# dedis/kyber

Measured on AMD Instinct MI355X. Metric: scalar-muls/s + pairings/s per node; MSM sec at 2^20 points, higher is better.
Workload: dtype int32 limbs (radix 2^25.5), int64 accumulate; 1 GPU; Ed25519 batched fixed-base + var-base scalar-mul, 2^20 scalars per GPU (BASELINE.json configs[1]); elements_per_gpu=1048576

## Files before the change

kyber_amd/csrc/ed25519.hip:

```cpp
#ifndef KYB_TU_WAVES
#define KYB_TU_WAVES 2
#endif
#include "context.h"
#include "ed25519_dev.cuh"
#include "ed25519_launch.h"
#include "msm.cuh"
#include "ed25519_h2c.cuh"
#include <stdlib.h>
#include <string.h>

#include <algorithm>
#include <atomic>
#include <chrono>
#include <thread>
#include <vector>

namespace kyb {


template <int G = 2>
__global__ void ed25519_build_base_table_kernel(int32_t* __restrict__ tab, const uint32_t* __restrict__ point,
                                                uint32_t* __restrict__ ok, int rows = ED_TAB_POS * ED_TAB_ENT) {
    const int t = blockIdx.x * blockDim.x + threadIdx.x;
    if (t >= rows) return;
    ge_p3 B;
    if (point) {
        uint32_t pw[8];
        load_words8(pw, point);
        const bool good = ge_p3_fromwords(B, pw);
        if (t == 0) *ok = good ? 1u : 0u;
    } else {
        B.X = fe_bx(); B.Y = fe_by(); fe_1(B.Z); B.T = fe_bt();
    }
    ed_comb_row<G>(tab + (size_t)t * ED_TAB_STRIDE, t, B);
}

__global__ __launch_bounds__(ED_ENC_BLOCK, KYB_TU_WAVES) void ed25519_encode_kernel(size_t n, const int32_t* __restrict__ proj,
                                                            const uint8_t* __restrict__ status,
                                                            uint32_t* __restrict__ out) {
    __shared__ int32_t pre_lds[EncPreLds<ED_ENC_BLOCK>::WORDS];
    static_assert(ED_ENC_BLOCK % 64 == 0 && sizeof(pre_lds) <= 80 * 1024 && sizeof(pre_lds) / (ED_ENC_BLOCK / 64) * 4 <= 160 * 1024,
                  "LDS: at least two blocks on a CU, and a wave on every SIMD");
    EncPreLds<ED_ENC_BLOCK> pre{pre_lds + threadIdx.x};
    ed_encode_chunk(n, proj, ed_encode_first(), blockDim.x, pre, [&](size_t i, uint32_t (&w)[8]) {
        if (status && status[i]) {
#pragma unroll
            for (int k = 0; k < 8; k++) w[k] = 0;
        }
        store_words8(out + i * 8, w);
    });
}


template <int G>
__global__ __launch_bounds__(256, 3) void ed25519_mul_base_kernel(
    size_t n, const uint32_t* __restrict__ scalars, uint32_t* __restrict__ out,
    const int32_t* __restrict__ tab, uint32_t flags, int32_t* __restrict__ proj) {
    const bool full = (flags & KYB_F_VARTIME) != 0;
    for (size_t idx = (size_t)blockIdx.x * blockDim.x + threadIdx.x; idx < n;
         idx += (size_t)gridDim.x * blockDim.x) {
        uint32_t a[8];
        load_words8(a, scalars + idx * 8);
        int8_t e[65];
        recode16(e, a, full);
        ge_p3 h;
        ge_p3_0(h);
        ge_precomp t;
        ge_p1p1 r;
        const int npos = full ? EdComb<G>::POS : EdComb<G>::POS_CT;
        EdCombDigits<G> digits(e);
#pragma unroll 1
        for (int k = 0; k < npos; k++) {
            const int d = digits.next(k);
            if (full && __ballot(d != 0) == 0) continue;
            select_precomp_tab<EdComb<G>::ENT>(t, tab, k, d);
            ge_madd(r, h, t);
            ge_p1p1_to_p3(h, r);
        }
        if (proj) {
            store_proj(proj, idx, h);
            continue;
        }
        uint32_t w[8];
        ge_p3_towords(w, h);
        store_words8(out + idx * 8, w);
    }
}

KYB_DEV void select_precomp_uniform(ge_precomp& t, const int32_t* __restrict__ tab, int i, int b) {
    const bool neg = b < 0;
    const int babs = neg ? -b : b;
    const int pos = i >> 1, mult = (i & 1) ? 16 : 1;
    fe_1(t.ypx);
    fe_1(t.ymx);
    fe_0(t.xy2d);
#pragma unroll 1
    for (int m = 1; m <= 8; m++) {
        const int4* e = reinterpret_cast<const int4*>(tab + (size_t)(pos * ED_TAB_ENT + (m * mult - 1)) * ED_TAB_STRIDE);
        int32_t w[32];
#pragma unroll
        for (int q = 0; q < 8; q++) {
            const int4 x = e[q];
            w[4 * q] = x.x;
            w[4 * q + 1] = x.y;
            w[4 * q + 2] = x.z;
            w[4 * q + 3] = x.w;
        }
        const int32_t keep = -(int32_t)(babs == m);
#pragma unroll
        for (int l = 0; l < 10; l++) {
            t.ypx.v[l] ^= (t.ypx.v[l] ^ w[l]) & keep;
            t.ymx.v[l] ^= (t.ymx.v[l] ^ w[10 + l]) & keep;
            t.xy2d.v[l] ^= (t.xy2d.v[l] ^ w[20 + l]) & keep;
        }
    }
    ge_precomp_cneg(t, neg);
}
__global__ __launch_bounds__(256, 3) void ed25519_mul_base_uniform_kernel(
    size_t n, const uint32_t* __restrict__ scalars, uint32_t* __restrict__ out,
    const int32_t* __restrict__ tab, int32_t* __restrict__ proj) {
    for (size_t idx = (size_t)blockIdx.x * blockDim.x + threadIdx.x; idx < n;
         idx += (size_t)gridDim.x * blockDim.x) {
        uint32_t a[8];
        load_words8(a, scalars + idx * 8);
        int8_t e[65];
        recode16(e, a, false);
        ge_p3 h;
        ge_p3_0(h);
        ge_precomp t;
        ge_p1p1 r;
        EdCombDigits<1> digits(e);
#pragma unroll 1
        for (int i = 0; i < 64; i++) {
            select_precomp_uniform(t, tab, i, digits.next(i));
            ge_madd(r, h, t);
            ge_p1p1_to_p3(h, r);
        }
        if (proj) {
            store_proj(proj, idx, h);
            continue;
        }
        uint32_t w[8];
        ge_p3_towords(w, h);
        store_words8(out + idx * 8, w);
    }
}


template <bool GTAB, bool UNI = false>
__global__ __launch_bounds__(128, 3) void ed25519_mul_kernel(
    size_t n, const uint32_t* __restrict__ scalars, const uint32_t* __restrict__ points,
    size_t points_stride, uint32_t* __restrict__ out, uint8_t* __restrict__ status,
    uint32_t flags, int32_t* __restrict__ proj, int4* __restrict__ gtab) {
    const size_t idx = (size_t)blockIdx.x * blockDim.x + threadIdx.x;
    if (idx >= n) return;
    const bool full = !UNI && (flags & KYB_F_VARTIME) != 0;
    uint32_t pw[8], a[8];
    load_words8(pw, points + idx * points_stride);
    load_words8(a, scalars + idx * 8);
    ge29_p3 A;
    const bool ok = ge_p3_fromwords(A, pw);
    int8_t e[65];
    recode16(e, a, full);
    ge29_p3 h;
    const int vt_top = full ? wave_top_digit(a) : 63;
    if constexpr (GTAB) {
        TabGlobal_t<fe29> tab{gtab + idx * 80};
        ge_scalarmult_w4<UNI, true>(h, e, A, full, tab, vt_top);
    } else {
        TabScratch_t<fe29> tab;
        ge_scalarmult_w4<UNI, true>(h, e, A, full, tab, vt_top);
    }
    if (proj) {
        store_proj(proj, idx, h);
        if (status) status[idx] = ok ? KYB_ST_OK : KYB_ST_BAD_POINT;
        return;
    }
    uint32_t w[8];
    ge_p3_towords(w, h);
    if (!ok) {
#pragma unroll
        for (int i = 0; i < 8; i++) w[i] = 0;
    }
    store_words8(out + idx * 8, w);
    if (status) status[idx] = ok ? KYB_ST_OK : KYB_ST_BAD_POINT;
}

int ed25519_build_tables(DeviceCtx* ctx) {
    KYB_HIP_CHECK(hipMalloc(&ctx->ed_base_tab, ED_TAB_WORDS * sizeof(int32_t)));
    hipLaunchKernelGGL(ed25519_build_base_table_kernel<2>, dim3((ED_TAB_POS * ED_TAB_ENT + 63) / 64), dim3(64), 0,
                       nullptr, ctx->ed_base_tab, (const uint32_t*)nullptr, (uint32_t*)nullptr, ED_TAB_POS * ED_TAB_ENT);
    KYB_HIP_CHECK(hipGetLastError());
    const auto t0 = std::chrono::steady_clock::now();
    KYB_HIP_CHECK(hipMalloc(&ctx->ed_wide_tab, ED_WIDE_WORDS * sizeof(int32_t)));
    hipLaunchKernelGGL(ed25519_build_base_table_kernel<ED_COMB_G>, dim3((EdWide::ROWS + 63) / 64), dim3(64), 0, nullptr,
                       ctx->ed_wide_tab, (const uint32_t*)nullptr, (uint32_t*)nullptr, EdWide::ROWS);
    KYB_HIP_CHECK(hipGetLastError());
    KYB_HIP_CHECK(hipStreamSynchronize(nullptr));
    ctx->ed_wide_build_us = std::chrono::duration_cast<std::chrono::microseconds>(std::chrono::steady_clock::now() - t0).count();
    return KYB_OK;
}
void ed25519_free_tables(DeviceCtx* ctx) {
    if (ctx->ed_base_tab) hipFree(ctx->ed_base_tab);
    if (ctx->ed_wide_tab) hipFree(ctx->ed_wide_tab);
    ctx->ed_base_tab = ctx->ed_wide_tab = nullptr;
}

constexpr size_t ENC_DEFER_MIN = 4096;


static int launch_mul_base(DeviceCtx* ctx, size_t n, const void* d_scalars, void* d_out, uint32_t flags,
                           hipStream_t st, const int32_t* tab = nullptr) {
    const bool wide = !tab && !(flags & KYB_F_UNIFORM);
    if (!tab) tab = wide ? ctx->ed_wide_tab : ctx->ed_base_tab;
    if (n == 0) return KYB_OK;
    const int block = 256;
    size_t want = (n + block - 1) / block;
    size_t cap = (size_t)ctx->num_cu * 8;
    int grid = (int)(want < cap ? want : cap);
    EdSlab w{};
    std::lock_guard<std::recursive_mutex> enq_lock(ctx->enq_mu);
    if (n >= ENC_DEFER_MIN)
        if (int rc = ed_slab(ctx, st, ED_SLAB_MUL_BASE, n, &w)) return rc;
    if (flags & KYB_F_UNIFORM) {
        hipLaunchKernelGGL(ed25519_mul_base_uniform_kernel, dim3(grid), dim3(block), 0, st, n,
                           (const uint32_t*)d_scalars, (uint32_t*)d_out, tab, w.proj);
    } else {
        const auto kernel = wide ? ed25519_mul_base_kernel<ED_COMB_G> : ed25519_mul_base_kernel<2>;
        hipLaunchKernelGGL(kernel, dim3(grid), dim3(block), 0, st, n, (const uint32_t*)d_scalars, (uint32_t*)d_out, tab,
                           flags, w.proj);
    }
    if (w.proj)
        hipLaunchKernelGGL(ed25519_encode_kernel, ed_encode_grid(n), dim3(ED_ENC_BLOCK), 0, st, n, w.proj,
                           (const uint8_t*)nullptr, (uint32_t*)d_out);
    KYB_HIP_CHECK(hipGetLastError());
    return KYB_OK;
}
static int launch_mul(size_t n, const void* d_scalars, const void* d_points, size_t stride, void* d_out,
                      void* d_status, uint32_t flags, hipStream_t st) {
    if (n == 0) return KYB_OK;
    const int block = 128;
    size_t grid = (n + block - 1) / block;
    EdSlab w{};
    uint8_t* stat = (uint8_t*)d_status;
    DeviceCtx* ctx;
    int rc = get_ctx(&ctx);
    if (rc) return rc;
    std::lock_guard<std::recursive_mutex> enq_lock(ctx->enq_mu);
    const bool defer = n >= ENC_DEFER_MIN, uni = (flags & KYB_F_UNIFORM) != 0;
    const auto kernel = defer ? (uni ? ed25519_mul_kernel<true, true> : ed25519_mul_kernel<true, false>)
                              : (uni ? ed25519_mul_kernel<false, true> : ed25519_mul_kernel<false, false>);
    if (defer) {
        if ((rc = ed_slab(ctx, st, ed_slab_mul(stat == nullptr), n, &w))) return rc;
        if (!stat) stat = w.status;
    }
    hipLaunchKernelGGL(kernel, dim3((unsigned)grid), dim3(block), 0, st, n, (const uint32_t*)d_scalars,
                       (const uint32_t*)d_points, stride, (uint32_t*)d_out, stat, flags, w.proj, w.gtab);
    if (w.proj)
        hipLaunchKernelGGL(ed25519_encode_kernel, ed_encode_grid(n), dim3(ED_ENC_BLOCK), 0, st, n, w.proj,
                           (const uint8_t*)stat, (uint32_t*)d_out);
    KYB_HIP_CHECK(hipGetLastError());
    return KYB_OK;
}

}

using namespace kyb;

static bool ed_mul_flags_bad(uint32_t flags) {
    return (flags & ~(KYB_F_VARTIME | KYB_F_UNIFORM)) || (flags & (KYB_F_VARTIME | KYB_F_UNIFORM)) == (KYB_F_VARTIME | KYB_F_UNIFORM);
}

extern "C" {

int kyb_ed25519_mul_base_dev(size_t n, const void* d_scalars, void* d_out, uint32_t flags, void* stream) {
    if ((n && (!d_scalars || !d_out)) || ed_mul_flags_bad(flags)) {
        set_error("kyb_ed25519_mul_base_dev: bad argument");
        return KYB_E_ARG;
    }
    DeviceCtx* ctx;
    int rc = get_ctx(&ctx);
    if (rc) return rc;
    return launch_mul_base(ctx, n, d_scalars, d_out, flags, (hipStream_t)stream);
}

int kyb_ed25519_mul_dev(size_t n, const void* d_scalars, const void* d_points, void* d_out, void* d_status,
                        uint32_t flags, void* stream) {
    if ((n && (!d_scalars || !d_points || !d_out)) || ed_mul_flags_bad(flags)) {
        set_error("kyb_ed25519_mul_dev: bad argument");
        return KYB_E_ARG;
    }
    DeviceCtx* ctx;
    int rc = get_ctx(&ctx);
    if (rc) return rc;
    return launch_mul(n, d_scalars, d_points, 8, d_out, d_status, flags, (hipStream_t)stream);
}

static int mul_host(size_t n, const uint8_t* scalars, const uint8_t* points, size_t stride, uint8_t* out,
                    uint8_t* status, uint32_t flags);

int kyb_ed25519_mul_base(size_t n, const uint8_t* scalars, uint8_t* out, uint32_t flags) {
    if ((n && (!scalars || !out)) || ed_mul_flags_bad(flags)) {
        set_error("kyb_ed25519_mul_base: bad argument");
        return KYB_E_ARG;
    }
    if (n == 0) return KYB_OK;
    if (md_active(n))
        return md_run(n, [&](int, size_t lo, size_t hi) { return kyb_ed25519_mul_base(hi - lo, scalars + 32 * lo, out + 32 * lo, flags); });
    return mul_host(n, scalars, nullptr, 0, out, nullptr, flags);
}

constexpr size_t PIPE_CHUNK_MAX = PIN_SLOT_ELEMS;
constexpr int PIPE_SLOTS = DeviceCtx::NPIN, PIPE_STREAMS = 3;
static size_t pipe_chunk(const DeviceCtx* ctx) {
    if (const char* e = getenv("KYB_PIPE_CHUNK")) {
        const size_t v = (size_t)strtoull(e, nullptr, 10) & ~size_t(63);
        if (v >= 4096) return std::min(PIPE_CHUNK_MAX, v);
    }
    (void)ctx;
    return size_t(1) << 17;
}
static int pipe_nstreams() {
    if (const char* e = getenv("KYB_PIPE_STREAMS")) {
        const int v = atoi(e);
        if (v >= 1 && v <= PIPE_STREAMS) return v;
// ... 466 lines not shown
```

kyber_amd/csrc/ed25519_consts.inc:

```
KYB_DEV fe fe_d() { return fe{{56195235, 13857412, 51736253, 6949390, 114729, 24766616, 60832955, 30306712, 48412415, 21499315}}; }
KYB_DEV fe fe_d2() { return fe{{45281625, 27714825, 36363642, 13898781, 229458, 15978800, 54557047, 27058993, 29715967, 9444199}}; }
KYB_DEV fe fe_sqrtm1() { return fe{{34513072, 25610706, 9377949, 3500415, 12389472, 33281959, 41962654, 31548777, 326685, 11406482}}; }
KYB_DEV fe fe_bx() { return fe{{52811034, 25909283, 16144682, 17082669, 27570973, 30858332, 40966398, 8378388, 20764389, 8758491}}; }
KYB_DEV fe fe_by() { return fe{{40265304, 26843545, 13421772, 20132659, 26843545, 6710886, 53687091, 13421772, 40265318, 26843545}}; }
KYB_DEV fe fe_bt() { return fe{{28827043, 27438313, 39759291, 244362, 8635006, 11264893, 19351346, 13413597, 16611511, 27139452}}; }
KYB_DEV fe fe_elligator_c1() { return fe{{54885894, 25242303, 55597453, 9067496, 51808079, 33312638, 25456129, 14121551, 54921728, 3972023}}; }
KYB_DEV fe fe_elligator_c2() { return fe{{34513073, 25610706, 9377949, 3500415, 12389472, 33281959, 41962654, 31548777, 326685, 11406482}}; }
```

kyber_amd/csrc/ed25519_dev.cuh:

```cuda
#pragma once
#include "ge25519.cuh"

#if !defined(__HIPCC__)
#include <type_traits>
struct int4 { int32_t x, y, z, w; };
struct uint4 { uint32_t x, y, z, w; };
inline int4 make_int4(int32_t x, int32_t y, int32_t z, int32_t w) { return int4{x, y, z, w}; }
inline uint4 make_uint4(uint32_t x, uint32_t y, uint32_t z, uint32_t w) { return uint4{x, y, z, w}; }
#define KYB_DEV_CONST static
#else
#define KYB_DEV_CONST __device__
#endif

namespace kyb {

constexpr int ED_TAB_POS = 33;
constexpr int ED_TAB_ENT = 136;
constexpr int ED_TAB_STRIDE = 32;
constexpr int ED_TAB_WORDS = ED_TAB_POS * ED_TAB_ENT * ED_TAB_STRIDE;

template <int G>
struct EdComb {
    static constexpr int POS = (65 + G - 1) / G;
    static constexpr int POS_CT = (64 + G - 1) / G;
    static constexpr int ENT = 8 * ((1 << (4 * G)) - 1) / 15;
    static constexpr int LAST_D = 65 - G * (POS - 1);
    static constexpr int LAST_ENT = 8 * ((1 << (4 * LAST_D)) - 1) / 15;
    static constexpr int ROWS = (POS - 1) * ENT + LAST_ENT;
};
#ifndef ED_COMB_G
#define ED_COMB_G 4
#endif
using EdWide = EdComb<ED_COMB_G>;
constexpr size_t ED_WIDE_WORDS = (size_t)EdWide::ROWS * ED_TAB_STRIDE;

KYB_DEV void load_words8(uint32_t w[8], const uint32_t* __restrict__ p) {
    const uint4 a = reinterpret_cast<const uint4*>(p)[0];
    const uint4 b = reinterpret_cast<const uint4*>(p)[1];
    w[0] = a.x; w[1] = a.y; w[2] = a.z; w[3] = a.w;
    w[4] = b.x; w[5] = b.y; w[6] = b.z; w[7] = b.w;
}
KYB_DEV void store_words8(uint32_t* __restrict__ p, const uint32_t w[8]) {
    reinterpret_cast<uint4*>(p)[0] = make_uint4(w[0], w[1], w[2], w[3]);
    reinterpret_cast<uint4*>(p)[1] = make_uint4(w[4], w[5], w[6], w[7]);
}

template <int G>
KYB_DEV void ed_comb_row(int32_t* __restrict__ o, int t, const ge_p3& B) {
    constexpr int ENT = EdComb<G>::ENT;
    const int pos = t / ENT, j = t - pos * ENT;
    ge_cached cB;
    ge_p3_to_cached(cB, B);
    ge_p3 acc;
    ge_p3_0(acc);
    ge_p1p1 r;
#pragma unroll 1
    for (int bit = 4 * G - 1; bit >= 0; bit--) {
        ge_dbl(r, acc.X, acc.Y, acc.Z);
        ge_p1p1_to_p3(acc, r);
        if (((j + 1) >> bit) & 1) {
            ge_add(r, acc, cB);
            ge_p1p1_to_p3(acc, r);
        }
    }
#pragma unroll 1
    for (int k = 0; k < 4 * G * pos; k++) {
        ge_dbl(r, acc.X, acc.Y, acc.Z);
        ge_p1p1_to_p3(acc, r);
    }
    fe zi, x, y, ypx, ymx, xy2d, z;
    fe_invert(zi, acc.Z);
    fe_mul(x, acc.X, zi);
    fe_mul(y, acc.Y, zi);
    fe_add(ypx, y, x);
    fe_sub(ymx, y, x);
    fe_mul(xy2d, x, y);
    fe_mul(xy2d, xy2d, fe_d2());
    fe_1(z);
    fe_mul(ypx, ypx, z);
    fe_mul(ymx, ymx, z);
#pragma unroll
    for (int l = 0; l < 10; l++) {
        o[l] = ypx.v[l];
        o[10 + l] = ymx.v[l];
        o[20 + l] = xy2d.v[l];
    }
    o[30] = o[31] = 0;
}

constexpr int ENC_CHUNK = 16;

KYB_DEV void store_proj(int32_t* __restrict__ proj, size_t idx, const ge_p3& h) {
    int32_t* o = proj + idx * 30;
#pragma unroll
    for (int l = 0; l < 10; l++) {
        o[l] = h.X.v[l];
        o[10 + l] = h.Y.v[l];
        o[20 + l] = h.Z.v[l];
    }
}
KYB_DEV void store_proj(int32_t* __restrict__ proj, size_t idx, const ge29_p3& h) {
    ge_p3 t;
    fe29_to_fe(t.X, h.X);
    fe29_to_fe(t.Y, h.Y);
    fe29_to_fe(t.Z, h.Z);
    store_proj(proj, idx, t);
}
KYB_DEV void load_fe(fe& f, const int32_t* __restrict__ p) {
#pragma unroll
    for (int l = 0; l < 10; l++) f.v[l] = p[l];
}
struct EncPreScratch {
    fe pre[ENC_CHUNK];
    KYB_DEV void put(int j, const fe& f) { pre[j] = f; }
    KYB_DEV void get(fe& f, int j) const { f = pre[j]; }
};
template <int LANES>
struct EncPreLds {
    int32_t* col;
    static constexpr int WORDS = ENC_CHUNK * 10 * LANES;
    KYB_DEV void put(int j, const fe& f) {
#pragma unroll
        for (int l = 0; l < 10; l++) col[(j * 10 + l) * LANES] = f.v[l];
    }
    KYB_DEV void get(fe& f, int j) const {
#pragma unroll
        for (int l = 0; l < 10; l++) f.v[l] = col[(j * 10 + l) * LANES];
        KYB_FE_MAG_SET(f, 1.01);
    }
};
#if defined(__HIPCC__)
template <int GROUP = 1>
KYB_DEV size_t ed_encode_first() {
    return (size_t)blockIdx.x * blockDim.x * (ENC_CHUNK / GROUP) + threadIdx.x;
}
#endif
template <int GROUP = 1, class Pre, class Emit>
KYB_DEV void ed_encode_chunk(size_t n, const int32_t* __restrict__ proj, size_t first, size_t stride, Pre& pre, Emit emit) {
    static_assert(GROUP >= 1 && GROUP <= ENC_CHUNK, "whole records per lane");
    int cnt = 0;
#pragma unroll
    for (int r = 0; r < ENC_CHUNK / GROUP; r++) cnt += (first + r * stride < n) ? GROUP : 0;
    if (cnt == 0) return;
    auto point = [&](int j) { return (first + (size_t)(j / GROUP) * stride) * GROUP + (size_t)(j % GROUP); };
    fe z, acc;
    load_fe(acc, proj + point(0) * 30 + 20);
    pre.put(0, acc);
#pragma unroll 1
    for (int j = 1; j < cnt; j++) {
        load_fe(z, proj + point(j) * 30 + 20);
        fe_mul(acc, acc, z);
        pre.put(j, acc);
    }
    fe inv;
    fe_invert(inv, acc);
#pragma unroll 1
    for (int j = cnt - 1; j >= 0; j--) {
        const size_t i = point(j);
        fe zi, X, Y;
        load_fe(z, proj + i * 30 + 20);
        if (j > 0) {
            pre.get(zi, j - 1);
            fe_mul(zi, inv, zi);
            fe_mul(inv, inv, z);
        } else {
            zi = inv;
        }
        load_fe(X, proj + i * 30);
        load_fe(Y, proj + i * 30 + 10);
        uint32_t w[8];
        ge_encode_with_zinv(w, X, Y, zi);
        emit(i, w);
    }
}

template <int ENT>
KYB_DEV void select_precomp_tab(ge_precomp& t, const int32_t* __restrict__ tab, int pos, int b) {
    const bool neg = b < 0;
    const int babs = neg ? -b : b;
    const int4* e = reinterpret_cast<const int4*>(tab + (size_t)(pos * ENT + (babs ? babs - 1 : 0)) * ED_TAB_STRIDE);
    int32_t w[32];
#pragma unroll
    for (int i = 0; i < 8; i++) {
        const int4 x = e[i];
        w[4 * i] = x.x;
        w[4 * i + 1] = x.y;
        w[4 * i + 2] = x.z;
        w[4 * i + 3] = x.w;
    }
#pragma unroll
    for (int l = 0; l < 10; l++) {
        t.ypx.v[l] = w[l];
        t.ymx.v[l] = w[10 + l];
        t.xy2d.v[l] = w[20 + l];
    }
    if (babs == 0) {
        fe_1(t.ypx);
        fe_1(t.ymx);
        fe_0(t.xy2d);
    }
    ge_precomp_cneg(t, neg);
}

KYB_DEV void ed_pack_digits(uint32_t pk[8], const int8_t e[65]) {
#pragma unroll
    for (int j = 0; j < 8; j++) {
        pk[j] = 0;
#pragma unroll
        for (int q = 0; q < 8; q++) pk[j] |= (uint32_t)((e[8 * j + q] + 8) & 15) << (4 * q);
    }
}

template <int G>
struct EdCombDigits {
    static_assert(G >= 1 && G <= 7, "a position's digits are read from one 32-bit word");
    static constexpr int PACKED = 63 / G;
    static constexpr int TAIL = EdComb<G>::POS - PACKED;
    uint32_t pk[8];
    int tail[TAIL];
    KYB_DEV explicit EdCombDigits(const int8_t e[65]) {
        ed_pack_digits(pk, e);
#pragma unroll
        for (int t = 0; t < TAIL; t++) {
            int d = 0;
#pragma unroll
            for (int i = G - 1; i >= 0; i--)
                if (G * (PACKED + t) + i <= 64) d = 16 * d + (int)e[G * (PACKED + t) + i];
            tail[t] = d;
        }
    }
    KYB_DEV int next(int k) {
        int d = (int)(pk[0] & ((1u << (4 * G)) - 1u)) - EdComb<G>::ENT;
#pragma unroll
        for (int j = 0; j < 7; j++) pk[j] = (pk[j] >> (4 * G)) | (pk[j + 1] << (32 - 4 * G));
        pk[7] >>= 4 * G;
#pragma unroll
        for (int t = 0; t < TAIL; t++)
            if (k == PACKED + t) d = tail[t];
        return d;
    }
};

template <class F = fe>
struct TabScratch_t {
    typedef typename ge_t<F>::cached cached;
    cached tab[8];
    KYB_DEV void put(int j, const cached& c) { tab[j] = c; }
    KYB_DEV void get(cached& c, int j) const { c = tab[j]; }
};
using TabScratch = TabScratch_t<>;
template <class F = fe>
struct TabGlobal_t;
using TabGlobal = TabGlobal_t<>;
template <>
struct TabGlobal_t<fe> {
    int4* base;
    KYB_DEV void put(int j, const ge_cached& c) {
        int4* q = base + j * 10;
        const fe* f[4] = {&c.YpX, &c.YmX, &c.Z, &c.T2d};
        int32_t w[40];
#pragma unroll
        for (int k = 0; k < 4; k++)
#pragma unroll
            for (int l = 0; l < 10; l++) w[10 * k + l] = f[k]->v[l];
#pragma unroll
        for (int i = 0; i < 10; i++) q[i] = make_int4(w[4 * i], w[4 * i + 1], w[4 * i + 2], w[4 * i + 3]);
    }
    KYB_DEV void get(ge_cached& c, int j) const {
        const int4* q = base + j * 10;
        int32_t w[40];
#pragma unroll
        for (int i = 0; i < 10; i++) {
            const int4 x = q[i];
            w[4 * i] = x.x;
            w[4 * i + 1] = x.y;
            w[4 * i + 2] = x.z;
            w[4 * i + 3] = x.w;
        }
        fe* f[4] = {&c.YpX, &c.YmX, &c.Z, &c.T2d};
#pragma unroll
        for (int k = 0; k < 4; k++)
#pragma unroll
            for (int l = 0; l < 10; l++) f[k]->v[l] = w[10 * k + l];
    }
    KYB_DEV void get_signed(ge_cached& c, int b) const;
};
KYB_DEV_CONST __attribute__((aligned(16))) const int32_t ED_CACHED_IDENTITY[40] = {1, 0, 0, 0, 0, 0, 0, 0, 0, 0,
                                                                               1, 0, 0, 0, 0, 0, 0, 0, 0, 0,
                                                                               1};
KYB_DEV void TabGlobal_t<fe>::get_signed(ge_cached& c, int b) const {
    const bool neg = b < 0;
    const int babs = neg ? -b : b;
#if defined(__HIPCC__)
    typedef int32_t i32x2 __attribute__((ext_vector_type(2)));
    typedef int32_t i32x4 __attribute__((ext_vector_type(4)));
    using gint = const __attribute__((address_space(1))) int32_t;
    using gint2 = const __attribute__((address_space(1))) i32x2;
    using gint4 = const __attribute__((address_space(1))) i32x4;
#else
    struct i32x2 { int32_t x, y; };
    struct i32x4 { int32_t x, y, z, w; };
    using gint = const int32_t;
    using gint2 = const i32x2;
    using gint4 = const i32x4;
#endif
    gint* e = babs ? (gint*)(base + (babs - 1) * 10) : (gint*)ED_CACHED_IDENTITY;
    gint2* p = (gint2*)(e + (neg ? 10 : 0));
    gint2* m = (gint2*)(e + (neg ? 0 : 10));
    gint4* q = (gint4*)(e + 20);
#pragma unroll
    for (int i = 0; i < 5; i++) {
        const i32x2 x = p[i], y = m[i];
        c.YpX.v[2 * i] = x.x;
        c.YpX.v[2 * i + 1] = x.y;
        c.YmX.v[2 * i] = y.x;
        c.YmX.v[2 * i + 1] = y.y;
    }
    int32_t w[20];
#pragma unroll
    for (int i = 0; i < 5; i++) {
        const i32x4 x = q[i];
        w[4 * i] = x.x;
        w[4 * i + 1] = x.y;
        w[4 * i + 2] = x.z;
        w[4 * i + 3] = x.w;
    }
    const int32_t s = -(int32_t)neg;
#pragma unroll
    for (int l = 0; l < 10; l++) {
        c.Z.v[l] = w[l];
        c.T2d.v[l] = (w[10 + l] ^ s) - s;
    }
}
template <>
struct TabGlobal_t<fe29> {
    int4* base;
    static constexpr int word(int field, int l) { return field < 2 ? (l < 8 ? 8 * field + l : 16 + field) : 18 + 9 * (field - 2) + l; }
    KYB_DEV void put(int j, const ge29_cached& c) {
        int4* q = base + j * 9;
        const fe29* f[4] = {&c.YpX, &c.YmX, &c.Z, &c.T2d};
        int32_t w[36];
#pragma unroll
        for (int k = 0; k < 4; k++)
#pragma unroll
            for (int l = 0; l < 9; l++) w[word(k, l)] = f[k]->v[l];
#pragma unroll
        for (int i = 0; i < 9; i++) q[i] = make_int4(w[4 * i], w[4 * i + 1], w[4 * i + 2], w[4 * i + 3]);
    }
    KYB_DEV void get(ge29_cached& c, int j) const {
        const int4* q = base + j * 9;
        int32_t w[36];
#pragma unroll
        for (int i = 0; i < 9; i++) {
            const int4 x = q[i];
            w[4 * i] = x.x;
            w[4 * i + 1] = x.y;
            w[4 * i + 2] = x.z;
            w[4 * i + 3] = x.w;
        }
        fe29* f[4] = {&c.YpX, &c.YmX, &c.Z, &c.T2d};
#pragma unroll
        for (int k = 0; k < 4; k++)
#pragma unroll
            for (int l = 0; l < 9; l++) f[k]->v[l] = w[word(k, l)];
        KYB_FE_MAG_SET(c.YpX, 3.001);
        KYB_FE_MAG_SET(c.YmX, 3.001);
        KYB_FE_MAG_SET(c.Z, 1.001);
        KYB_FE_MAG_SET(c.T2d, 1.001);
    }
    KYB_DEV void get_signed(ge29_cached& c, int b) const;
};
KYB_DEV_CONST __attribute__((aligned(16))) const int32_t ED_CACHED_IDENTITY29[36] = {1, 0, 0, 0, 0, 0, 0, 0,
                                                                                 1, 0, 0, 0, 0, 0, 0, 0,
                                                                                 0, 0, 1};
KYB_DEV void TabGlobal_t<fe29>::get_signed(ge29_cached& c, int b) const {
    const bool neg = b < 0;
    const int babs = neg ? -b : b;
#if defined(__HIPCC__)
    typedef int32_t i32x4 __attribute__((ext_vector_type(4)));
    using gint = const __attribute__((address_space(1))) int32_t;
    using gint4 = const __attribute__((address_space(1))) i32x4;
#else
    struct i32x4 { int32_t x, y, z, w; };
    using gint = const int32_t;
    using gint4 = const i32x4;
#endif
    gint* e = babs ? (gint*)(base + (babs - 1) * 9) : (gint*)ED_CACHED_IDENTITY29;
    gint4* p = (gint4*)(e + (neg ? 8 : 0));
    gint4* m = (gint4*)(e + (neg ? 0 : 8));
    gint4* q = (gint4*)(e + 16);
#pragma unroll
    for (int i = 0; i < 2; i++) {
        const i32x4 x = p[i], y = m[i];
        c.YpX.v[4 * i] = x.x;
        c.YpX.v[4 * i + 1] = x.y;
        c.YpX.v[4 * i + 2] = x.z;
        c.YpX.v[4 * i + 3] = x.w;
        c.YmX.v[4 * i] = y.x;
        c.YmX.v[4 * i + 1] = y.y;
        c.YmX.v[4 * i + 2] = y.z;
        c.YmX.v[4 * i + 3] = y.w;
    }
    int32_t w[20];
#pragma unroll
    for (int i = 0; i < 5; i++) {
        const i32x4 x = q[i];
        w[4 * i] = x.x;
        w[4 * i + 1] = x.y;
        w[4 * i + 2] = x.z;
        w[4 * i + 3] = x.w;
    }
    c.YpX.v[8] = neg ? w[1] : w[0];
    c.YmX.v[8] = neg ? w[0] : w[1];
    const int32_t s = -(int32_t)neg;
#pragma unroll
    for (int l = 0; l < 9; l++) {
        c.Z.v[l] = w[2 + l];
        c.T2d.v[l] = (w[11 + l] ^ s) - s;
    }
    KYB_FE_MAG_SET(c.YpX, 3.001);
    KYB_FE_MAG_SET(c.YmX, 3.001);
    KYB_FE_MAG_SET(c.Z, 1.001);
    KYB_FE_MAG_SET(c.T2d, 1.001);
}
template <bool UNI = false, class C, class Tab>
KYB_DEV void select_cached(C& c, const Tab& tab, int b) {
    typedef decltype(c.Z) F;
    const bool neg = b < 0;
    const int babs = neg ? -b : b;
    if constexpr (UNI) {
        ge_cached_0(c);
#pragma unroll 1
        for (int m = 1; m <= 8; m++) {
            C x;
            tab.get(x, m - 1);
            const int32_t keep = -(int32_t)(babs == m);
#pragma unroll
            for (int l = 0; l < F::N; l++) {
                c.YpX.v[l] ^= (c.YpX.v[l] ^ x.YpX.v[l]) & keep;
                c.YmX.v[l] ^= (c.YmX.v[l] ^ x.YmX.v[l]) & keep;
                c.Z.v[l] ^= (c.Z.v[l] ^ x.Z.v[l]) & keep;
                c.T2d.v[l] ^= (c.T2d.v[l] ^ x.T2d.v[l]) & keep;
            }
        }
    } else if constexpr (std::is_same_v<Tab, TabGlobal_t<F>>) {
        tab.get_signed(c, b);
        return;
    } else {
        tab.get(c, babs ? babs - 1 : 0);
        if (babs == 0) ge_cached_0(c);
    }
    ge_cached_cneg(c, neg);
}

KYB_DEV int wave_top_digit(const uint32_t a[8]) {
    int bits = 0;
#pragma unroll
    for (int i = 0; i < 8; i++)
        if (a[i]) bits = 32 * i + 32 - __builtin_clz(a[i]);
    int t = (bits + 3) >> 2;
    if (t > 64) t = 64;
#if defined(__HIP_DEVICE_COMPILE__)
#pragma unroll
    for (int off = 32; off >= 1; off >>= 1) {
        const int o = __shfl_xor(t, off, 64);
        t = o > t ? o : t;
    }
    t = __builtin_amdgcn_readfirstlane(t);
#endif
    return t;
}

template <bool AFFINE = false, class P3, class Tab>
KYB_DEV void ge_window_table(Tab& tab, const P3& A) {
    typedef ge_t<decltype(A.X)> G;
    typename G::p1p1 t;
    P3 u;
    typename G::cached c;
    ge_p3_to_cached(c, A);
    tab.put(0, c);
    if constexpr (AFFINE) {
        const typename G::precomp a{c.YpX, c.YmX, c.T2d};
        u = A;
#pragma unroll 1
        for (int i = 0; i < 7; i++) {
            ge_madd(t, u, a);
            ge_p1p1_to_p3(u, t);
            ge_p3_to_cached(c, u);
            tab.put(i + 1, c);
        }
    } else {
#pragma unroll 1
        for (int i = 0; i < 7; i++) {
            ge_add(t, A, c);
            ge_p1p1_to_p3(u, t);
            ge_p3_to_cached(c, u);
            tab.put(i + 1, c);
        }
    }
}

template <bool UNI = false, bool AFFINE = false, class P3, class Tab>
KYB_DEV void ge_scalarmult_w4(P3& h, const int8_t e[65], const P3& A, bool full, Tab& tab, int vt_top) {
    typedef ge_t<decltype(A.X)> G;
    typename G::p1p1 t;
    P3 u;
    typename G::p2 r;
    typename G::cached c;
    ge_window_table<AFFINE>(tab, A);
    ge_p3_0(u);
    int top = 63;
    if (full) top = vt_top;
    select_cached<UNI>(c, tab, e[top]);
    ge_add(t, u, c);
    uint32_t pk[8];
    ed_pack_digits(pk, e);
    auto shl4 = [&pk]() {
#pragma unroll
        for (int j = 7; j > 0; j--) pk[j] = (pk[j] << 4) | (pk[j - 1] >> 28);
        pk[0] <<= 4;
    };
#pragma unroll 1
    for (int i = top; i < 64; i++) shl4();
#pragma unroll 1
    for (int i = top - 1; i >= 0; i--) {
        const int d = (int)(pk[7] >> 28) - 8;
        shl4();
        ge_p1p1_to_p2(r, t);
        ge_dbl(t, r.X, r.Y, r.Z);
        ge_p1p1_to_p2(r, t);
        ge_dbl(t, r.X, r.Y, r.Z);
        ge_p1p1_to_p2(r, t);
        ge_dbl(t, r.X, r.Y, r.Z);
        ge_p1p1_to_p2(r, t);
        ge_dbl(t, r.X, r.Y, r.Z);
#if defined(__HIP_DEVICE_COMPILE__)
        if (!UNI && full && __ballot(d != 0) == 0) continue;
#endif
        ge_p1p1_to_p3(u, t);
        select_cached<UNI>(c, tab, d);
        ge_add(t, u, c);
    }
    ge_p1p1_to_p3(h, t);
}

}
```

kyber_amd/csrc/ge25519.cuh:

```cuda
#pragma once
#include "fe25519.cuh"
#include "fe29.cuh"

namespace kyb {

struct ge_p2 { fe X, Y, Z; };
struct ge_p3 { fe X, Y, Z, T; };
struct ge_p1p1 { fe X, Y, Z, T; };
struct ge_cached { fe YpX, YmX, Z, T2d; };
struct ge_precomp { fe ypx, ymx, xy2d; };
struct ge29_p2 { fe29 X, Y, Z; };
struct ge29_p3 { fe29 X, Y, Z, T; };
struct ge29_p1p1 { fe29 X, Y, Z, T; };
struct ge29_cached { fe29 YpX, YmX, Z, T2d; };
struct ge29_precomp { fe29 ypx, ymx, xy2d; };
template <class F> struct ge_t;
template <> struct ge_t<fe> {
    typedef ge_p2 p2; typedef ge_p3 p3; typedef ge_p1p1 p1p1; typedef ge_cached cached; typedef ge_precomp precomp;
};
template <> struct ge_t<fe29> {
    typedef ge29_p2 p2; typedef ge29_p3 p3; typedef ge29_p1p1 p1p1; typedef ge29_cached cached; typedef ge29_precomp precomp;
};

#include "ed25519_consts.inc"
#include "ed25519_consts29.inc"
template <class F> struct fe_k;
template <> struct fe_k<fe> {
    static KYB_DEV fe d() { return fe_d(); }
    static KYB_DEV fe d2() { return fe_d2(); }
    static KYB_DEV fe sqrtm1() { return fe_sqrtm1(); }
};
template <> struct fe_k<fe29> {
    static KYB_DEV fe29 d() { return fe29_d(); }
    static KYB_DEV fe29 d2() { return fe29_d2(); }
    static KYB_DEV fe29 sqrtm1() { return fe29_sqrtm1(); }
};

template <class P3>
KYB_DEV void ge_p3_0(P3& h) {
    fe_0(h.X);
    fe_1(h.Y);
    fe_1(h.Z);
    fe_0(h.T);
}
template <class C>
KYB_DEV void ge_cached_0(C& c) {
    fe_1(c.YpX);
    fe_1(c.YmX);
    fe_1(c.Z);
    fe_0(c.T2d);
}
template <class P2, class P1>
KYB_DEV void ge_p1p1_to_p2(P2& r, const P1& p) {
    fe_mul(r.X, p.X, p.T);
    fe_mul(r.Y, p.Y, p.Z);
    fe_mul(r.Z, p.Z, p.T);
}
template <class P3, class P1>
KYB_DEV void ge_p1p1_to_p3(P3& r, const P1& p) {
    fe_mul(r.X, p.X, p.T);
    fe_mul(r.Y, p.Y, p.Z);
    fe_mul(r.Z, p.Z, p.T);
    fe_mul(r.T, p.X, p.Y);
}
template <class C, class P3>
KYB_DEV void ge_p3_to_cached(C& r, const P3& p) {
    fe_add(r.YpX, p.Y, p.X);
    fe_sub(r.YmX, p.Y, p.X);
    r.Z = p.Z;
    fe_mul(r.T2d, p.T, fe_k<decltype(p.T)>::d2());
}
template <class P1, class F>
KYB_DEV void ge_dbl(P1& r, const F& X, const F& Y, const F& Z) {
    F t0;
    fe_sq(r.X, X);
    fe_sq(r.Z, Y);
    fe_sq2(r.T, Z);
    fe_add(r.Y, X, Y);
    fe_sq(t0, r.Y);
    fe_add(r.Y, r.Z, r.X);
    fe_sub(r.Z, r.Z, r.X);
    fe_sub(r.X, t0, r.Y);
    fe_sub(r.T, r.T, r.Z);
}
template <class P1, class P3, class C>
KYB_DEV void ge_add(P1& r, const P3& p, const C& q) {
    decltype(p.X) t0;
    fe_add(r.X, p.Y, p.X);
    fe_sub(r.Y, p.Y, p.X);
    fe_mul(r.Z, r.X, q.YpX);
    fe_mul(r.Y, r.Y, q.YmX);
    fe_mul(r.T, q.T2d, p.T);
    fe_mul(r.X, p.Z, q.Z);
    fe_add(t0, r.X, r.X);
    fe_sub(r.X, r.Z, r.Y);
    fe_add(r.Y, r.Z, r.Y);
    fe_add(r.Z, t0, r.T);
    fe_sub(r.T, t0, r.T);
}
template <class P1, class P3, class C>
KYB_DEV void ge_madd(P1& r, const P3& p, const C& q) {
    decltype(p.X) t0;
    fe_add(r.X, p.Y, p.X);
    fe_sub(r.Y, p.Y, p.X);
    fe_mul(r.Z, r.X, q.ypx);
    fe_mul(r.Y, r.Y, q.ymx);
    fe_mul(r.T, q.xy2d, p.T);
    fe_add(t0, p.Z, p.Z);
    fe_sub(r.X, r.Z, r.Y);
    fe_add(r.Y, r.Z, r.Y);
    fe_add(r.Z, t0, r.T);
    fe_sub(r.T, t0, r.T);
}
template <class C>
KYB_DEV void ge_cached_cneg(C& c, bool neg) {
    fe_cswap(c.YpX, c.YmX, neg);
    decltype(c.T2d) nt;
    fe_neg(nt, c.T2d);
    fe_cmov(c.T2d, nt, neg);
}
KYB_DEV void ge_precomp_cneg(ge_precomp& c, bool neg) {
    fe_cswap(c.ypx, c.ymx, neg);
    fe nt;
    fe_neg(nt, c.xy2d);
    fe_cmov(c.xy2d, nt, neg);
}

template <class F>
KYB_DEV void ge_encode_with_zinv(uint32_t w[8], const F& X, const F& Y, const F& zinv) {
    F x, y;
    fe_mul(x, X, zinv);
    fe_mul(y, Y, zinv);
    fe_towords(w, y);
    w[7] ^= (uint32_t)fe_isnegative(x) << 31;
}
template <class P3>
KYB_DEV void ge_p3_towords(uint32_t w[8], const P3& p) {
    decltype(p.Z) zi;
    fe_invert(zi, p.Z);
    ge_encode_with_zinv(w, p.X, p.Y, zi);
}
template <class P3>
KYB_DEV bool ge_p3_fromwords(P3& p, const uint32_t w[8]) {
    typedef decltype(p.X) F;
    F u, v, v3, vxx, check;
    fe_fromwords(p.Y, w);
    fe_1(p.Z);
    fe_sq(u, p.Y);
    fe_mul(v, u, fe_k<F>::d());
    fe_sub(u, u, p.Z);
    fe_add(v, v, p.Z);
    fe_sq(v3, v);
    fe_mul(v3, v3, v);
    fe_sq(p.X, v3);
    fe_mul(p.X, p.X, v);
    fe_mul(p.X, p.X, u);
    fe_pow22523(p.X, p.X);
    fe_mul(p.X, p.X, v3);
    fe_mul(p.X, p.X, u);
    fe_sq(vxx, p.X);
    fe_mul(vxx, vxx, v);
    fe_sub(check, vxx, u);
    bool ok = true;
    if (fe_isnonzero(check)) {
        fe_add(check, vxx, u);
        ok = !fe_isnonzero(check);
        F xs;
        fe_mul(xs, p.X, fe_k<F>::sqrtm1());
        p.X = xs;
    }
    const bool sign = (w[7] >> 31) != 0;
    F nx;
    fe_neg(nx, p.X);
    fe_cmov(p.X, nx, fe_isnegative(p.X) != sign);
    fe_mul(p.T, p.X, p.Y);
    return ok;
}

KYB_DEV void recode16(int8_t e[65], const uint32_t a[8], bool full256) {
    int carry = 0;
#pragma unroll
    for (int i = 0; i < 64; i++) {
        int d = (int)((a[i >> 3] >> ((i & 7) * 4)) & 15) + carry;
        if (i < 63) {
            carry = (d + 8) >> 4;
            d -= carry << 4;
        }
        e[i] = (int8_t)d;
    }
    int top = e[63];
    int c2 = 0;
    if (full256) {
        c2 = (top + 8) >> 4;
        top -= c2 << 4;
    } else if (top > 8) {
        top = 0;
    }
    e[63] = (int8_t)top;
    e[64] = (int8_t)c2;
}

KYB_DEV bool ed_effective_scalar(uint32_t (&k)[8]) {
    uint32_t c = 0, t7 = 0;
#pragma unroll
    for (int j = 0; j < 8; j++) {
        const uint64_t s = (uint64_t)k[j] + (j < 7 ? 0x88888888u : 0x08888888u) + c;
        t7 = (uint32_t)s;
        c = (uint32_t)(s >> 32);
    }
    const uint32_t e63 = (c << 4) | (t7 >> 28);
    if (e63 <= 8) return false;
    const uint32_t carried = e63 - (k[7] >> 28);
    k[7] &= 0x0fffffffu;
    if (!carried) return false;
    uint32_t b = 0;
#pragma unroll
    for (int j = 0; j < 8; j++) {
        const uint64_t d = (uint64_t)(j == 7 ? 0x10000000u : 0u) - k[j] - b;
        k[j] = (uint32_t)d;
        b = (uint32_t)(d >> 63);
    }
    return true;
}

}
```

kyber_amd/csrc/gen_consts.py:

```python
#!/usr/bin/env python3
import os

HERE = os.path.dirname(os.path.abspath(__file__))


def limbs_25_5(x):
    out, off = [], 0
    for i in range(10):
        w = 25 if i & 1 else 26
        out.append((x >> off) & ((1 << w) - 1))
        off += w
    assert off == 255 and x >> 255 == 0
    return out


def ed25519():
    p = 2**255 - 19
    d = (-121665 * pow(121666, p - 2, p)) % p
    sqrtm1 = pow(2, (p - 1) // 4, p)
    by = 4 * pow(5, p - 2, p) % p
    u, v = (by * by - 1) % p, (d * by * by + 1) % p
    bx = (u * pow(v, 3, p) * pow(u * pow(v, 7, p) % p, (p - 5) // 8, p)) % p
    if (v * bx * bx - u) % p:
        bx = bx * sqrtm1 % p
    assert (v * bx * bx - u) % p == 0
    if bx & 1:
        bx = p - bx
    a = (-486664) % p
    c1 = pow(a, (p + 3) // 8, p)
    if c1 * c1 % p != a:
        c1 = c1 * sqrtm1 % p
    assert c1 * c1 % p == a
    if c1 & 1:
        c1 = p - c1
    c2 = pow(2, (p + 3) // 8, p)
    consts = dict(d=d, d2=2 * d % p, sqrtm1=sqrtm1, bx=bx, by=by, bt=bx * by % p, elligator_c1=c1, elligator_c2=c2)
    lines = ["// generated by gen_consts.py -- do not edit"]
    for name, val in consts.items():
        ls = ", ".join(str(v) for v in limbs_25_5(val))
        lines.append(f"KYB_DEV fe fe_{name}() {{ return fe{{{{{ls}}}}}; }}")
    open(os.path.join(HERE, "ed25519_consts.inc"), "w").write("\n".join(lines) + "\n")
    lines = ["// generated by gen_consts.py -- do not edit"]
    for name in ("d", "d2", "sqrtm1"):
        ls = ", ".join(str(v) for v in _limbs(consts[name], 9, 29))
        lines.append(f"KYB_DEV fe29 fe29_{name}() {{ return fe29{{{{{ls}}}}}; }}")
    open(os.path.join(HERE, "ed25519_consts29.inc"), "w").write("\n".join(lines) + "\n")


def _limbs(x, n, w):
    assert x >> (n * w) == 0
    return [(x >> (w * i)) & ((1 << w) - 1) for i in range(n)]


def _words(x, nw):
    assert x >> (32 * nw) == 0
    return [(x >> (32 * i)) & 0xFFFFFFFF for i in range(nw)]


def _arr(vals):
    return "{" + ", ".join("0x%xu" % v for v in vals) + "}"


class MontField:
    def __init__(self, p, n, w, nwords):
        self.p, self.n, self.w, self.nwords = p, n, w, nwords
        self.R = 1 << (n * w)
        assert self.R > 4 * p and 32 * nwords <= n * w

    def mont(self, x):
        return _words(x % self.p * self.R % self.p, self.nwords)

    def mont2(self, c):
        return "{" + _arr(self.mont(c[0])) + ", " + _arr(self.mont(c[1])) + "}"

    def emit(self, name, extra=""):
        p, n, w = self.p, self.n, self.w
        ninv = (-pow(p, -1, 1 << w)) % (1 << w)
        nw = self.nwords
        L = [f"struct {name} {{",
             f"    static constexpr int N = {n}, W = {w}, NWORDS = {nw}, PBITS = {p.bit_length()};",
             f"    static constexpr uint32_t P[N] = {_arr(_limbs(p, n, w))};  // limbs (multiplier internals)",
             f"    static constexpr uint32_t PW[NWORDS] = {_arr(_words(p, nw))};  // words",
             f"    static constexpr uint32_t NINV = 0x{ninv:x}u;",
             f"    static constexpr uint32_t ONE[NWORDS] = {_arr(self.mont(1))};",
             f"    static constexpr uint32_t R2[NWORDS] = {_arr(_words(self.R * self.R % p, nw))};",
             f"    static constexpr uint32_t PM2[NWORDS] = {_arr(_words(p - 2, nw))};  // p - 2",
             f"    static constexpr uint32_t HALF[NWORDS] = {_arr(_words((p - 1) // 2, nw))};  // (p - 1) / 2, plain",
             ]
        if p % 4 == 3:
            L.append(f"    static constexpr uint32_t SQRT_EXP[NWORDS] = {_arr(_words((p + 1) // 4, nw))};  // (p + 1) / 4")
            L.append(f"    static constexpr int SQRT_BITS = {((p + 1) // 4).bit_length()};")
            L.append(f"    static constexpr uint32_t PM3D4[NWORDS] = {_arr(_words((p - 3) // 4, nw))};  // (p - 3) / 4")
            L.append(f"    static constexpr uint32_t INV2[NWORDS] = {_arr(self.mont(pow(2, -1, p)))};  // 1/2 (Montgomery)")
        if extra:
            L.append(extra)
        L.append("};")
        return "\n".join(L)


def _f2_mul(a, b, p):
    return ((a[0] * b[0] - a[1] * b[1]) % p, (a[0] * b[1] + a[1] * b[0]) % p)


def _f2_pow(a, e, p):
    r = (1, 0)
    while e:
        if e & 1:
            r = _f2_mul(r, a, p)
        a = _f2_mul(a, a, p)
        e >>= 1
    return r


def _f2_inv(a, p):
    n = pow(a[0] * a[0] + a[1] * a[1], -1, p)
    return (a[0] * n % p, -a[1] * n % p)


def bls12381():
    x = -0xD201000000010000
    r = x**4 - x**2 + 1
    p = (x - 1) ** 2 * r // 3 + x
    assert p == 0x1A0111EA397FE69A4B1BA7B6434BACD764774B84F38512BF6730D2A0F6B0F6241EABFFFEB153FFFFB9FEFFFFFFFFAAAB
    F = MontField(p, 13, 30, 12)
    g1 = (0x17F1D3A73197D7942695638C4FA9AC0FC3688C4F9774B905A14E3A3F171BAC586C55E83FF97A1AEFFB3AF00ADB22C6BB,
          0x08B3F481E3AAA0F1A09E30ED741D8AE4FCF5E095D5D00AF600DB18CB2C04B3EDD03CC744A2888AE40CAA232946C5E7E1)
    g2 = ((0x024AA2B2F08F0A91260805272DC51051C6E47AD4FA403B02B4510B647AE3D1770BAC0326A805BBEFD48056C8C121BDB8,
           0x13E02B6052719F607DACD3A088274F65596BD0D09920B61AB5DA61BBDC7F5049334CF11213945D57E5AC7D055D042B7E),
          (0x0CE5D527727D6E118CC9CDC6DA2E351AADFD9BAA8CBDD3A76D429A695160D12C923AC9CC3BACA289E193548608B82801,
           0x0606C4A02EA734CC32ACD2B02BC28B99CB3E287E85A763AF267492AB572E99AB3F370D275CEC1DA1AAA9075FF05F79BE))
    assert (g1[1] ** 2 - g1[0] ** 3 - 4) % p == 0
    xi = (1, 1)
    beta = pow(2, (p - 1) // 3, p)
    assert pow(beta, 3, p) == 1 and beta != 1
    cx = _f2_inv(_f2_pow(xi, (p - 1) // 3, p), p)
    cy = _f2_inv(_f2_pow(xi, (p - 1) // 2, p), p)
    out = ["// generated by gen_consts.py -- do not edit", "#pragma once", "#include <stdint.h>", "namespace kyb {",
           F.emit("Bls12381Fp"),
           "struct Bls12381Tower {", "    typedef Bls12381Fp F;", "    static constexpr int XI0 = 1;",
           "    static constexpr bool LAZY12 = true;  // R/p = 2^9: three levels of lazy Karatsuba sums (tower.cuh)",
           "};",
           "struct Bls12381Curve {",
           "    typedef Bls12381Tower T;",
           "    static constexpr uint64_t X_ABS = 0xd201000000010000ull;  // the curve parameter is -X_ABS",
           f"    static constexpr uint32_t B1[12] = {_arr(F.mont(4))};",
           f"    static constexpr uint32_t B2[2][12] = {F.mont2((4, 4))};",
           f"    static constexpr uint32_t G1X[12] = {_arr(F.mont(g1[0]))};",
           f"    static constexpr uint32_t G1Y[12] = {_arr(F.mont(g1[1]))};",
           f"    static constexpr uint32_t G2X[2][12] = {F.mont2(g2[0])};",
           f"    static constexpr uint32_t G2Y[2][12] = {F.mont2(g2[1])};",
           f"    static constexpr uint32_t BETA[12] = {_arr(F.mont(beta))};",
           f"    static constexpr uint32_t PSI_CX[2][12] = {F.mont2(cx)};",
           f"    static constexpr uint32_t PSI_CY[2][12] = {F.mont2(cy)};",
           f"    static constexpr uint32_t R_WORDS[8] = {_arr(_words(r, 8))};  // group order r",
           "};", "}  // namespace kyb", ""]
    open(os.path.join(HERE, "bls12381_params.h"), "w").write("\n".join(out))


def _bn(tag, u, xi0, g1, g2, doc, strict, svdw=None):
    p = 36 * u**4 + 36 * u**3 + 24 * u**2 + 6 * u + 1
    F = MontField(p, 9, 29, 8)
    xi = (xi0, 1)
    twist_b = _f2_mul((3, 0), _f2_inv(xi, p), p)
    n = 36 * u ** 4 + 36 * u ** 3 + 18 * u ** 2 + 6 * u + 1
    lam = 36 * u ** 3 + 18 * u ** 2 + 6 * u + 1
    assert (lam * lam + lam + 1) % n == 0

    def add(P, Q):
        if P is None: return Q
        if Q is None: return P
        if P[0] == Q[0]:
            if (P[1] + Q[1]) % p == 0: return None
            m = 3 * P[0] * P[0] * pow(2 * P[1], -1, p) % p
        else:
            m = (Q[1] - P[1]) * pow(Q[0] - P[0], -1, p) % p
        x = (m * m - P[0] - Q[0]) % p
        return (x, (m * (P[0] - x) - P[1]) % p)

    acc, base, e = None, g1, lam
    while e:
        if e & 1: acc = add(acc, base)
        base = add(base, base); e >>= 1
    beta = None
    for g in range(2, 50):
        c = pow(g, (p - 1) // 3, p)
        if c != 1:
            for cand in (c, c * c % p):
                if acc == (cand * g1[0] % p, g1[1]): beta = cand
            break
# ... 124 lines not shown
```

Before: 194.7 million scalar-muls/s.

## Skip identity-point first additions and trailing p3 conversion in Ed25519 scalar-mul

```diff
diff --git a/kyber_amd/csrc/ed25519.hip b/kyber_amd/csrc/ed25519.hip
--- a/kyber_amd/csrc/ed25519.hip
+++ b/kyber_amd/csrc/ed25519.hip
@@ -64,19 +64,7 @@
         int8_t e[65];
         recode16(e, a, full);
         ge_p3 h;
-        ge_p3_0(h);
-        ge_precomp t;
-        ge_p1p1 r;
-        const int npos = full ? EdComb<G>::POS : EdComb<G>::POS_CT;
-        EdCombDigits<G> digits(e);
-#pragma unroll 1
-        for (int k = 0; k < npos; k++) {
-            const int d = digits.next(k);
-            if (full && __ballot(d != 0) == 0) continue;
-            select_precomp_tab<EdComb<G>::ENT>(t, tab, k, d);
-            ge_madd(r, h, t);
-            ge_p1p1_to_p3(h, r);
-        }
+        ed_comb_walk<G>(h, e, full, tab);
         if (proj) {
             store_proj(proj, idx, h);
             continue;
@@ -126,12 +114,13 @@
         int8_t e[65];
         recode16(e, a, false);
         ge_p3 h;
-        ge_p3_0(h);
         ge_precomp t;
         ge_p1p1 r;
         EdCombDigits<1> digits(e);
+        select_precomp_uniform(t, tab, 0, digits.next(0));
+        ge_precomp_to_p3(h, t);
 #pragma unroll 1
-        for (int i = 0; i < 64; i++) {
+        for (int i = 1; i < 64; i++) {
             select_precomp_uniform(t, tab, i, digits.next(i));
             ge_madd(r, h, t);
             ge_p1p1_to_p3(h, r);
@@ -162,15 +151,17 @@
     const bool ok = ge_p3_fromwords(A, pw);
     int8_t e[65];
     recode16(e, a, full);
-    ge29_p3 h;
+    ge29_p1p1 t;
     const int vt_top = full ? wave_top_digit(a) : 63;
     if constexpr (GTAB) {
         TabGlobal_t<fe29> tab{gtab + idx * 80};
-        ge_scalarmult_w4<UNI, true>(h, e, A, full, tab, vt_top);
+        ge_scalarmult_w4_p1p1<UNI, true>(t, e, A, full, tab, vt_top);
     } else {
         TabScratch_t<fe29> tab;
-        ge_scalarmult_w4<UNI, true>(h, e, A, full, tab, vt_top);
-    }
+        ge_scalarmult_w4_p1p1<UNI, true>(t, e, A, full, tab, vt_top);
+    }
+    ge29_p2 h;
+    ge_p1p1_to_p2(h, t);
     if (proj) {
         store_proj(proj, idx, h);
         if (status) status[idx] = ok ? KYB_ST_OK : KYB_ST_BAD_POINT;
diff --git a/kyber_amd/csrc/ed25519_consts.inc b/kyber_amd/csrc/ed25519_consts.inc
--- a/kyber_amd/csrc/ed25519_consts.inc
+++ b/kyber_amd/csrc/ed25519_consts.inc
@@ -6,3 +6,4 @@
 KYB_DEV fe fe_bt() { return fe{{28827043, 27438313, 39759291, 244362, 8635006, 11264893, 19351346, 13413597, 16611511, 27139452}}; }
 KYB_DEV fe fe_elligator_c1() { return fe{{54885894, 25242303, 55597453, 9067496, 51808079, 33312638, 25456129, 14121551, 54921728, 3972023}}; }
 KYB_DEV fe fe_elligator_c2() { return fe{{34513073, 25610706, 9377949, 3500415, 12389472, 33281959, 41962654, 31548777, 326685, 11406482}}; }
+KYB_DEV fe fe_dinv() { return fe{{30013507, 3972531, 42321084, 12719050, 2979674, 28954470, 51415654, 29910370, 18959708, 16925179}}; }
diff --git a/kyber_amd/csrc/ed25519_dev.cuh b/kyber_amd/csrc/ed25519_dev.cuh
--- a/kyber_amd/csrc/ed25519_dev.cuh
+++ b/kyber_amd/csrc/ed25519_dev.cuh
@@ -99,12 +99,15 @@
         o[20 + l] = h.Z.v[l];
     }
 }
-KYB_DEV void store_proj(int32_t* __restrict__ proj, size_t idx, const ge29_p3& h) {
+KYB_DEV void store_proj(int32_t* __restrict__ proj, size_t idx, const ge29_p2& h) {
     ge_p3 t;
     fe29_to_fe(t.X, h.X);
     fe29_to_fe(t.Y, h.Y);
     fe29_to_fe(t.Z, h.Z);
     store_proj(proj, idx, t);
+}
+KYB_DEV void store_proj(int32_t* __restrict__ proj, size_t idx, const ge29_p3& h) {
+    store_proj(proj, idx, ge29_p2{h.X, h.Y, h.Z});
 }
 KYB_DEV void load_fe(fe& f, const int32_t* __restrict__ p) {
 #pragma unroll
@@ -240,6 +243,26 @@
         return d;
     }
 };
+
+template <int G>
+KYB_DEV void ed_comb_walk(ge_p3& h, const int8_t e[65], bool full, const int32_t* __restrict__ tab) {
+    ge_precomp t;
+    ge_p1p1 r;
+    const int npos = full ? EdComb<G>::POS : EdComb<G>::POS_CT;
+    EdCombDigits<G> digits(e);
+    select_precomp_tab<EdComb<G>::ENT>(t, tab, 0, digits.next(0));
+    ge_precomp_to_p3(h, t);
+#pragma unroll 1
+    for (int k = 1; k < npos; k++) {
+        const int d = digits.next(k);
+#if defined(__HIP_DEVICE_COMPILE__)
+        if (full && __ballot(d != 0) == 0) continue;
+#endif
+        select_precomp_tab<EdComb<G>::ENT>(t, tab, k, d);
+        ge_madd(r, h, t);
+        ge_p1p1_to_p3(h, r);
+    }
+}
 
 template <class F = fe>
 struct TabScratch_t {
@@ -500,19 +523,22 @@
     }
 }
 
-template <bool UNI = false, bool AFFINE = false, class P3, class Tab>
-KYB_DEV void ge_scalarmult_w4(P3& h, const int8_t e[65], const P3& A, bool full, Tab& tab, int vt_top) {
+template <bool UNI = false, bool AFFINE = false, class P1, class P3, class Tab>
+KYB_DEV void ge_scalarmult_w4_p1p1(P1& t, const int8_t e[65], const P3& A, bool full, Tab& tab, int vt_top) {
     typedef ge_t<decltype(A.X)> G;
-    typename G::p1p1 t;
+    constexpr bool EARLY = !UNI && std::is_same_v<Tab, TabGlobal_t<fe29>>;
     P3 u;
     typename G::p2 r;
     typename G::cached c;
     ge_window_table<AFFINE>(tab, A);
-    ge_p3_0(u);
     int top = 63;
     if (full) top = vt_top;
     select_cached<UNI>(c, tab, e[top]);
-    ge_add(t, u, c);
+    if (top == 0) {
+        ge_cached_to_p1p1(t, c);
+        return;
+    }
+    ge_dbl_cached(t, c);
     uint32_t pk[8];
     ed_pack_digits(pk, e);
     auto shl4 = [&pk]() {
@@ -523,24 +549,34 @@
 #pragma unroll 1
     for (int i = top; i < 64; i++) shl4();
 #pragma unroll 1
-    for (int i = top - 1; i >= 0; i--) {
+    for (int i = top - 1;; i--) {
         const int d = (int)(pk[7] >> 28) - 8;
         shl4();
+        if constexpr (EARLY) select_cached<UNI>(c, tab, d);
         ge_p1p1_to_p2(r, t);
         ge_dbl(t, r.X, r.Y, r.Z);
         ge_p1p1_to_p2(r, t);
         ge_dbl(t, r.X, r.Y, r.Z);
         ge_p1p1_to_p2(r, t);
         ge_dbl(t, r.X, r.Y, r.Z);
+        bool add = true;
+#if defined(__HIP_DEVICE_COMPILE__)
+        if (!UNI && full && __ballot(d != 0) == 0) add = false;
+#endif
+        if (add) {
+            ge_p1p1_to_p3(u, t);
+            if constexpr (!EARLY) select_cached<UNI>(c, tab, d);
+            ge_add(t, u, c);
+        }
+        if (i == 0) break;
         ge_p1p1_to_p2(r, t);
         ge_dbl(t, r.X, r.Y, r.Z);
-#if defined(__HIP_DEVICE_COMPILE__)
-        if (!UNI && full && __ballot(d != 0) == 0) continue;
-#endif
-        ge_p1p1_to_p3(u, t);
-        select_cached<UNI>(c, tab, d);
-        ge_add(t, u, c);
-    }
+    }
+}
+template <bool UNI = false, bool AFFINE = false, class P3, class Tab>
+KYB_DEV void ge_scalarmult_w4(P3& h, const int8_t e[65], const P3& A, bool full, Tab& tab, int vt_top) {
+    typename ge_t<decltype(A.X)>::p1p1 t;
+    ge_scalarmult_w4_p1p1<UNI, AFFINE>(t, e, A, full, tab, vt_top);
     ge_p1p1_to_p3(h, t);
 }
 
diff --git a/kyber_amd/csrc/ge25519.cuh b/kyber_amd/csrc/ge25519.cuh
--- a/kyber_amd/csrc/ge25519.cuh
+++ b/kyber_amd/csrc/ge25519.cuh
@@ -82,6 +82,44 @@
     fe_sub(r.Z, r.Z, r.X);
     fe_sub(r.X, t0, r.Y);
     fe_sub(r.T, r.T, r.Z);
+}
+template <class F>
+KYB_DEV void ge_cached_xy(F& X, F& Y, const F& YpX, const F& YmX) {
+#pragma unroll
+    for (int l = 0; l < F::N; l++) {
+        X.v[l] = (YpX.v[l] - YmX.v[l]) >> 1;
+        Y.v[l] = (YpX.v[l] + YmX.v[l]) >> 1;
+    }
+    KYB_FE_MAG_SET(X, KYB_FE_MAG(YpX) > KYB_FE_MAG(YmX) ? KYB_FE_MAG(YpX) : KYB_FE_MAG(YmX));
+    KYB_FE_MAG_SET(Y, KYB_FE_MAG(X));
+}
+template <class P1, class C>
+KYB_DEV void ge_dbl_cached(P1& r, const C& q) {
+    decltype(q.Z) x, y, t0;
+    ge_cached_xy(x, y, q.YpX, q.YmX);
+    fe_sq(r.X, x);
+    fe_sq(r.Z, y);
+    fe_sq2(r.T, q.Z);
+    fe_sq(t0, q.YpX);
+    fe_add(r.Y, r.Z, r.X);
+    fe_sub(r.Z, r.Z, r.X);
+    fe_sub(r.X, t0, r.Y);
+    fe_sub(r.T, r.T, r.Z);
+}
+template <class P1, class C>
+KYB_DEV void ge_cached_to_p1p1(P1& r, const C& q) {
+    ge_cached_xy(r.X, r.Y, q.YpX, q.YmX);
+    r.Z = q.Z;
+    r.T = q.Z;
+}
+template <class P3, class C>
+KYB_DEV void ge_precomp_to_p3(P3& r, const C& q) {
+    fe_sub(r.X, q.ypx, q.ymx);
+    fe_add(r.Y, q.ypx, q.ymx);
+    fe_0(r.Z);
+    r.Z.v[0] = 2;
+    KYB_FE_MAG_SET(r.Z, 2.0 / (1 << 25));
+    fe_mul(r.T, q.xy2d, fe_dinv());
 }
 template <class P1, class P3, class C>
 KYB_DEV void ge_add(P1& r, const P3& p, const C& q) {
diff --git a/kyber_amd/csrc/gen_consts.py b/kyber_amd/csrc/gen_consts.py
--- a/kyber_amd/csrc/gen_consts.py
+++ b/kyber_amd/csrc/gen_consts.py
@@ -34,7 +34,8 @@
     if c1 & 1:
         c1 = p - c1
     c2 = pow(2, (p + 3) // 8, p)
-    consts = dict(d=d, d2=2 * d % p, sqrtm1=sqrtm1, bx=bx, by=by, bt=bx * by % p, elligator_c1=c1, elligator_c2=c2)
+    consts = dict(d=d, d2=2 * d % p, sqrtm1=sqrtm1, bx=bx, by=by, bt=bx * by % p, elligator_c1=c1, elligator_c2=c2,
+                  dinv=pow(d, p - 2, p))
     lines = ["// generated by gen_consts.py -- do not edit"]
     for name, val in consts.items():
         ls = ", ".join(str(v) for v in limbs_25_5(val))
```

Measured after the change: 197.4 million scalar-muls/s (median of 6 runs). 1.01x the previous value.
